# xds0112/5G_based_System_level_Integrated_Sensing_and_Communication_Simulator

Hardware: AMD Instinct MI355X
Metric: sensing slots/sec (CDL echo->2D-FFT->2D-CFAR) (higher is better)
Workload: dtype f64

## Files before the change

5g_based_system_level_integrated_sensing_and_communication_simulator_amd/_build.py:

```python
from __future__ import annotations

import os
import subprocess
import sys
from concurrent.futures import ThreadPoolExecutor

HERE = os.path.dirname(os.path.abspath(__file__))
CSRC = os.path.join(HERE, "csrc")
OBJ = os.path.join(CSRC, "build")
LIB = os.path.join(HERE, "libisac_hip.so")
SOURCES = ["capi.hip", "fft2d.hip", "tables.hip", "echo.hip", "rdm.hip", "cov.hip", "eigh.hip", "music.hip", "cdl.hip", "cdl_os.hip", "cqi.hip", "los.hip", "doa2d.hip", "doa.hip", "rxfe.hip", "targets.hip", "cfar.hip"]
HEADERS = ["isac_common.hpp", "isac_internal.hpp", "cut_window.hpp", "fft_lds.hpp", "echo_dev.hpp", "eigh_dev.hpp", "eigh_layout.hpp", os.path.join("..", "..", "include", "isac.h"), os.path.join("..", "..", "include", "isac_targets.h"), os.path.join("..", "..", "include", "isac_cfar.h"), os.path.join("..", "..", "include", "isac_cfar_mc.h")]
HIPCC = os.environ.get("HIPCC", "/opt/rocm/bin/hipcc")
FLAGS = ["--offload-arch=gfx950", "-O3", "-std=c++17", "-fPIC", "-fno-gpu-rdc", "-Wall", "-Wno-unused-function",
         "-Wno-unused-variable", "-Wno-unused-value", "-Wno-unused-result", "-ffp-contract=on"]


def _newer(target: str, deps: list[str]) -> bool:
    if not os.path.exists(target):
        return False
    t = os.path.getmtime(target)
    return all(os.path.getmtime(d) <= t for d in deps if os.path.exists(d))


def _compile(src: str, force: bool) -> str:
    obj = os.path.join(OBJ, os.path.splitext(src)[0] + ".o")
    deps = [os.path.join(CSRC, src)] + [os.path.join(CSRC, h) for h in HEADERS] + [os.path.abspath(__file__)]
    if not force and _newer(obj, deps):
        return obj
    cmd = [HIPCC, *FLAGS, "-c", os.path.join(CSRC, src), "-o", obj]
    r = subprocess.run(cmd, capture_output=True, text=True)
    if r.returncode != 0:
        raise RuntimeError(f"hipcc failed for {src}:\n{r.stdout}\n{r.stderr}")
    if r.stderr.strip():
        sys.stderr.write(r.stderr)
    return obj


def build(force: bool = False, verbose: bool = False) -> str:
    os.makedirs(OBJ, exist_ok=True)
    srcs = [s for s in SOURCES if os.path.exists(os.path.join(CSRC, s))]
    with ThreadPoolExecutor(max_workers=min(len(srcs), os.cpu_count() or 4)) as ex:
        objs = list(ex.map(lambda s: _compile(s, force), srcs))
    if force or not _newer(LIB, objs):
        cmd = [HIPCC, "--offload-arch=gfx950", "-shared", "-fPIC", "-o", LIB, *objs,
               "-Wl,-soname,libisac_hip.so", "-Wl,--no-undefined"]
        r = subprocess.run(cmd, capture_output=True, text=True)
        if r.returncode != 0:
            raise RuntimeError(f"link failed:\n{r.stdout}\n{r.stderr}")
    if verbose:
        print(f"built {LIB}")
    return LIB


if __name__ == "__main__":
    build(force="--force" in sys.argv, verbose=True)
```

5g_based_system_level_integrated_sensing_and_communication_simulator_amd/csrc/echo.hip:

```cpp
#include <cstring>
#include <type_traits>

#include "isac_internal.hpp"
#include "fft_lds.hpp"
#include "echo_dev.hpp"

namespace isac {

template <int QT, int UNROLL>
__device__ __forceinline__ void beam_sample(const c64* __restrict__ p , long long T, int A, const c64* __restrict__ s_steer , c64 (&acc)[QT]) {
#pragma unroll
  for (int q = 0; q < QT; ++q) acc[q] = mk(0.0, 0.0);
  int a = 0;
  for (; a + UNROLL <= A; a += UNROLL) {
    c64 v[UNROLL];
#pragma unroll
    for (int u = 0; u < UNROLL; ++u) v[u] = p[(long long)(a + u) * T];
#pragma unroll
    for (int u = 0; u < UNROLL; ++u)
#pragma unroll
      for (int q = 0; q < QT; ++q) acc[q] = fma(v[u], s_steer[q * A + a + u], acc[q]);
  }
  for (; a < A; ++a) {
    c64 v = p[(long long)a * T];
#pragma unroll
    for (int q = 0; q < QT; ++q) acc[q] = fma(v, s_steer[q * A + a], acc[q]);
  }
}

template <int QT, int UNROLL>
__global__ __launch_bounds__(256) void beamsum_kernel(const c64* __restrict__ tx, long long T, int A,
                                                      const c64* __restrict__ steer ,
                                                      c64* __restrict__ beam ) {
  extern __shared__ __attribute__((aligned(16))) char smem_raw[];
  c64* s_steer = reinterpret_cast<c64*>(smem_raw);
  for (int i = threadIdx.x; i < A * QT; i += blockDim.x) s_steer[i] = steer[i];
  __syncthreads();
  for (long long t0 = (long long)blockIdx.x * 256; t0 < T; t0 += (long long)gridDim.x * 256) {
    const long long t = t0 + threadIdx.x;
    const long long tc = t < T ? t : T - 1;
    c64 acc[QT];
    beam_sample<QT, UNROLL>(tx + tc, T, A, s_steer, acc);
    if (t < T) {
#pragma unroll
      for (int q = 0; q < QT; ++q) beam[(long long)q * T + t] = acc[q];
    }
  }
}

struct TargetDesc {
  double wd;
  double lsf;
  long long shift;
};
constexpr int kMaxTargets = 64;
struct TargetTable {
  TargetDesc t[kMaxTargets];
};

__device__ __forceinline__ c64 rx_phase(double w , double tt) {
  double s, c;
  sincos(w * tt, &s, &c);
  return mk(c, -s);
}

__device__ __forceinline__ c64 coef_value(c64 b, long long t, const TargetDesc& td, double w, double Ts, double tt, c64 prx) {
  double sd, cd, st, ct;
  sincos(td.wd * tt, &sd, &cd);
  sincos(w * ((double)(t - td.shift) * Ts), &st, &ct);
  c64 v = b * mk(ct, st);
  v = v * mk(cd, sd);
  v = v * td.lsf;
  return v * prx;
}

__global__ __launch_bounds__(256) void coef_kernel(const c64* __restrict__ beam, long long T, int Q,
                                                   TargetTable tab, double w , double Ts,
                                                   c64* __restrict__ coef ,
                                                   c64* __restrict__ phase_rx ) {
  long long t = (long long)blockIdx.x * blockDim.x + threadIdx.x;
  if (t >= T) return;
  double tt = (double)t * Ts;
  c64 prx = rx_phase(w, tt);
  phase_rx[t] = prx;
  for (int q = 0; q < Q; ++q) {
    long long d = tab.t[q].shift;
    c64 out = mk(0.0, 0.0);
    if (t >= d) out = coef_value(beam[(long long)q * T + (t - d)], t, tab.t[q], w, Ts, tt, prx);
    coef[(long long)q * T + t] = out;
  }
}

template <int QT>
struct CoefTargets {
  TargetDesc t[QT];
};
template <int QT, int UNROLL>
__global__ __launch_bounds__(256) void beamsum_coef_kernel(const c64* __restrict__ tx, long long T, int A,
                                                           const c64* __restrict__ steer ,
                                                           CoefTargets<QT> tab, double w , double Ts,
                                                           c64* __restrict__ coef ) {
  extern __shared__ __attribute__((aligned(16))) char smem_raw[];
  c64* s_steer = reinterpret_cast<c64*>(smem_raw);
  for (int i = threadIdx.x; i < A * QT; i += blockDim.x) s_steer[i] = steer[i];
  __syncthreads();
  for (long long t0 = (long long)blockIdx.x * 256; t0 < T; t0 += (long long)gridDim.x * 256) {
    const long long u = t0 + threadIdx.x;
    const long long uc = u < T ? u : T - 1;
    c64 acc[QT];
    beam_sample<QT, UNROLL>(tx + uc, T, A, s_steer, acc);
#pragma unroll
    for (int q = 0; q < QT; ++q) {
      const long long d = tab.t[q].shift, t = u + d;
      c64* cq = coef + (long long)q * T;
      if (u < d && u < T) cq[u] = mk(0.0, 0.0);
      if (u < T && t >= 0 && t < T) {
        const double tt = (double)t * Ts;
        cq[t] = coef_value(acc[q], t, tab.t[q], w, Ts, tt, rx_phase(w, tt));
      }
    }
  }
}

__global__ __launch_bounds__(256) void radar_waveform_kernel(long long T, int A, int Q, const c64* __restrict__ coef,
                                                             const c64* __restrict__ steer_rq ,
                                                             const c64* __restrict__ phase_rx, int noise_mode,
                                                             const c64* __restrict__ noise, double n0s, uint64_t seed,
                                                             c64* __restrict__ rx) {
  long long t = (long long)blockIdx.x * blockDim.x + threadIdx.x;
  int r = blockIdx.y;
  if (t >= T) return;
  rx[t + T * r] = rx_sample(t, r, T, Q, coef, steer_rq + (long long)r * Q, phase_rx, noise_mode, noise, n0s, seed);
}

struct OfdmGeom {
  int nfft, n_sc, cp_base, cp_long, sym_per_half;
};

template <class FFT, bool SYNTH, int QT = 0>
__global__ __launch_bounds__(256, 2) void demod_kernel(OfdmGeom g, long long T, int A, int L_whole, int L_out,
                                                       const c64* __restrict__ tw,
                                                       int Q_rt, const c64* __restrict__ coef,
                                                       const c64* __restrict__ steer_rq, const c64* __restrict__ phase_rx,
                                                       int noise_mode, const c64* __restrict__ noise, double n0s,
                                                       uint64_t seed,
                                                       const c64* __restrict__ wave,
                                                       c64* __restrict__ grid, const c64* __restrict__ logtab_g) {
  extern __shared__ __attribute__((aligned(16))) char smem_raw[];
  c64* lds = reinterpret_cast<c64*>(smem_raw);
  const int tid = threadIdx.x;
  FFT fft;
  constexpr bool kTables = SYNTH && QT > 0 && std::is_same<FFT, Fft4096>::value;
  const int Q = QT ? QT : Q_rt;
  {
    const int col = blockIdx.x;
    const int l = col % L_whole, r = col / L_whole;
    const int cp = cp_of_symbol(l, g.cp_base, g.cp_long, g.sym_per_half);
    const int off = cp / 2;
    const long long w0 = symbol_start(l, g.nfft, g.cp_base, g.cp_long, g.sym_per_half) + off;
    const int dshift = cp - off;
    if constexpr (SYNTH) {
      const c64* sr = steer_rq + (long long)r * Q;
      if (noise_mode == ISAC_NOISE_PHILOX) {
        if constexpr (kTables) {
          c64* lt = lds + FFT::LDS_ELEMS;
          if (tid < kLogTabSize) lt[tid] = logtab_g[tid];
          fft.init_table(lds, tw, tid);
          const c64* w256 = lds + FFT::IMG;
          fft.template fill<4>([&](int n) { return rx_sample(w0 + n, r, T, Q, coef, sr, phase_rx, ISAC_NOISE_PHILOX, noise, n0s, seed, w256, lt); }, tid);
          fft.init_twiddles(tw, tid);
        } else {
          fft.template fill<4>([&](int n) { return rx_sample(w0 + n, r, T, Q, coef, sr, phase_rx, ISAC_NOISE_PHILOX, noise, n0s, seed); }, tid);
        }
      } else {
        const int nm = (noise_mode == ISAC_NOISE_INJECTED) ? ISAC_NOISE_INJECTED : ISAC_NOISE_NONE;
        fft.template fill<8>([&](int n) { return rx_sample(w0 + n, r, T, Q, coef, sr, phase_rx, nm, noise, n0s, seed); }, tid);
      }
    } else {
      const c64* src = wave + w0 + T * (long long)r;
      fft.fill([&](int n) { return src[n]; }, tid);
    }
    if (!(kTables && noise_mode == ISAC_NOISE_PHILOX)) fft.init(lds, tw, tid);
    fft.template transform<-1>(lds, tw, tid);
    c64* dst = grid + (long long)g.n_sc * ((long long)l + (long long)L_out * r);
    const int half = g.n_sc / 2;
    fft.drain(
        [&](int k, c64 v) {
          const int kb = (k < g.nfft / 2) ? k : k - g.nfft;
          const int row = kb + half;
          const c64 ph = fft.phase_ramp(lds, tw, kb, dshift);
          if (row >= 0 && row < g.n_sc) {
            const c64 o = v * ph;
            __builtin_nontemporal_store(o.re, &dst[row].re);
            __builtin_nontemporal_store(o.im, &dst[row].im);
          }
        },
        tid);
  }
}

template <int QT, int NZ>
// ... 225 lines not shown
  }
}

__global__ __launch_bounds__(256) void mod_window_kernel(OfdmGeom g, ModIo io, int A, int L, const c64* __restrict__ head,
                                                         const double* __restrict__ rise, c64* __restrict__ wave) {
  const long long i = (long long)blockIdx.x * blockDim.x + threadIdx.x;
  const long long n = (long long)io.n_win * L * A;
  if (i >= n) return;
  const int w = (int)(i % io.n_win), l = (int)((i / io.n_win) % L), a = (int)(i / ((long long)io.n_win * L));
  const long long e = symbol_start(io.sym0 + l + 1, g.nfft, g.cp_base, g.cp_long, g.sym_per_half) -
                      symbol_start(io.sym0, g.nfft, g.cp_base, g.cp_long, g.sym_per_half);
  c64* p = wave + io.t_off + io.wave_rows * (long long)a + e - io.n_win + w;
  const c64 hv = head[(long long)io.n_win * ((long long)((l + 1) % L) + (long long)L * a) + w];
  *p = *p * rise[io.n_win - 1 - w] + hv;
}

__global__ __launch_bounds__(256) void copy_slot_kernel(const c64* __restrict__ src , c64* __restrict__ dst, int K, int L, int A,
                                                        int grid_cols, int l_off) {
  const long long i = (long long)blockIdx.x * blockDim.x + threadIdx.x;
  const long long n = (long long)K * L * A;
  if (i >= n) return;
  const long long k = i % K, l = (i / K) % L, a = i / ((long long)K * L);
  dst[k + (long long)K * ((l_off + l) + (long long)grid_cols * a)] = src ? src[i] : mk(0.0, 0.0);
}

__global__ __launch_bounds__(256) void synth_qpsk_kernel(c64* __restrict__ grid, int K, int L, int A, uint64_t seed,
                                                         int zero_s_slots) {
  long long i = (long long)blockIdx.x * blockDim.x + threadIdx.x;
  long long n = (long long)K * L * A;
  if (i >= n) return;
  int l = (int)((i / K) % L);
  int slot = l / 14;
  c64 v = mk(0.0, 0.0);
  if (!(zero_s_slots && (slot % 4) == 3)) {
    uint32_t o[4];
    philox4x32_10((uint32_t)i, (uint32_t)((uint64_t)i >> 32), 1u, 0u, (uint32_t)seed, (uint32_t)(seed >> 32), o);
    v = mk((o[0] & 1u) ? kR2 : -kR2, (o[1] & 1u) ? kR2 : -kR2);
  }
  grid[i] = v;
}

}

using namespace isac;

static int check_carrier(isac_ctx* ctx, const isac_carrier* c) {
  if (!c) return fail(ctx, ISAC_ERR_INVALID_ARG, "carrier is NULL");
  if (c->nfft < 128 || c->nfft > 4096 || (c->nfft & (c->nfft - 1)))
    return fail(ctx, ISAC_ERR_UNSUPPORTED, "carrier.nfft must be a power of two in 128..4096: no integral normal cyclic prefix (144 Nfft / 2048 samples) exists below 128");
  if (c->n_sc <= 0 || c->n_sc > c->nfft || (c->n_sc & 1)) return fail(ctx, ISAC_ERR_INVALID_ARG, "carrier.n_sc invalid");
  if (c->scs_khz != 15 && c->scs_khz != 30 && c->scs_khz != 60 && c->scs_khz != 120)
    return fail(ctx, ISAC_ERR_INVALID_ARG, "carrier.scs_khz must be 15/30/60/120");
  return ISAC_OK;
}

static OfdmGeom geom_of(const isac_carrier* c) {
  Numerology n = numerology(c->nfft, c->scs_khz);
  return OfdmGeom{c->nfft, c->n_sc, n.cp_base, n.cp_long, n.sym_per_half};
}

static int whole_symbols(const OfdmGeom& g, long long T) {
  long long lo = 0, hi = T / g.nfft + 1;
  while (lo < hi) {
    long long mid = (lo + hi + 1) / 2;
    if (symbol_start((int)mid, g.nfft, g.cp_base, g.cp_long, g.sym_per_half) <= T) lo = mid; else hi = mid - 1;
  }
  return (int)lo;
}

extern "C" int isac_ofdm_symbol_count(const isac_carrier* carrier, int64_t T, int32_t* n_symbols) {
  if (!carrier || !n_symbols || T < 0) return ISAC_ERR_INVALID_ARG;
  *n_symbols = whole_symbols(geom_of(carrier), T);
  return ISAC_OK;
}

extern "C" int isac_ofdm_waveform_length(const isac_carrier* carrier, int32_t L, int64_t* T) {
  if (!carrier || !T || L < 0) return ISAC_ERR_INVALID_ARG;
  OfdmGeom g = geom_of(carrier);
  *T = symbol_start(L, g.nfft, g.cp_base, g.cp_long, g.sym_per_half);
  return ISAC_OK;
}

static int prepare_echo(isac_ctx* ctx, const c64* d_tx, long long T, const isac_radar_channel_params* rp,
                        const uint8_t* los, int* q_out, bool coef_only = false) {
  if (!d_tx || !rp || !los) return fail(ctx, ISAC_ERR_INVALID_ARG, "NULL argument");
  if (T <= 0 || rp->n_ants <= 0 || rp->n_targets < 0) return fail(ctx, ISAC_ERR_INVALID_ARG, "bad T / n_ants / n_targets");
  ctx->lazy.valid = false;
  if (!(rp->fs > 0)) return fail(ctx, ISAC_ERR_INVALID_ARG, "fs must be positive");
  const int A = rp->n_ants;
  const double c0 = 299792458.0;
  const double lambda = c0 / rp->fc;
  const double Ts = 1.0 / rp->fs;
  const double two_pi = 2.0 * M_PI;
  TargetTable tab{};
  std::vector<c64> steer_aq;
  int Q = 0;
  for (int i = 0; i < rp->n_targets; ++i) {
    if (los[i] != 1) continue;
    if (Q >= kMaxTargets) return fail(ctx, ISAC_ERR_CAPACITY, "more than 64 LoS targets");
    for (int a = 0; a < A; ++a) {
      const isac_c64 sv = rp->rx_steering[(size_t)a + (size_t)A * i];
      steer_aq.push_back(mk(sv.re, sv.im));
    }
    double path_delay = 2.0 * rp->range[i] / c0;
    tab.t[Q].shift = (long long)std::ceil(path_delay / Ts);
    double fd = 2.0 * rp->velocity[i] / lambda;
    tab.t[Q].wd = two_pi * fd;
    tab.t[Q].lsf = rp->large_scale_fading[i];
    ++Q;
  }
  if (Q == 0) return fail(ctx, ISAC_ERR_NO_LOS, "no LoS target: rxWaveform is empty (basicRadarChannel.m:59,64)");
  std::vector<c64> steer_rq((size_t)A * Q);
  for (int q = 0; q < Q; ++q)
    for (int a = 0; a < A; ++a) steer_rq[(size_t)a * Q + q] = steer_aq[(size_t)q * A + a];
  ISAC_TRY(ensure(ctx, ctx->steer, sizeof(c64) * (size_t)A * Q * 2));
  ISAC_TRY(ensure(ctx, ctx->beam, sizeof(c64) * (size_t)Q * T));
  ISAC_TRY(ensure(ctx, ctx->coef, sizeof(c64) * (size_t)Q * T));
  ISAC_TRY(ensure(ctx, ctx->phase_rx, sizeof(c64) * (size_t)T));
  c64* d_steer_aq = (c64*)ctx->steer.p;
  {
    const size_t bytes = sizeof(c64) * (size_t)A * Q * 2;
    void* hst = nullptr;
    ISAC_TRY(stage_acquire(ctx, bytes, &hst));
    std::memcpy(hst, steer_aq.data(), bytes / 2);
    std::memcpy((char*)hst + bytes / 2, steer_rq.data(), bytes / 2);
    ISAC_TRY(stage_commit(ctx, d_steer_aq, bytes));
  }
  const unsigned gb = cdiv(T, 256);
  const unsigned gbs = (unsigned)std::min<long long>(gb, 1024);
  timeline_mark(ctx, 0, ctx->stream);
  const double w = two_pi * rp->fc;
  if (coef_only && Q <= 2) {
    auto launch = [&](auto qc) {
      constexpr int QT = decltype(qc)::value;
      CoefTargets<QT> ct;
      for (int q = 0; q < QT; ++q) ct.t[q] = tab.t[q];
      hipLaunchKernelGGL((beamsum_coef_kernel<QT, 32>), dim3(gbs), dim3(256), sizeof(c64) * A * QT, ctx->stream, d_tx, T, A, (const c64*)d_steer_aq, ct, w, Ts, (c64*)ctx->coef.p);
    };
    if (Q == 1) launch(std::integral_constant<int, 1>{});
    else launch(std::integral_constant<int, 2>{});
    ISAC_HIP(hipGetLastError());
    timeline_mark(ctx, 1, ctx->stream);
    *q_out = Q;
    return ISAC_OK;
  }
#define ISAC_BEAMSUM(QT) \
  hipLaunchKernelGGL((beamsum_kernel<QT, (QT <= 2 ? 32 : 8)>), dim3(gbs), dim3(256), sizeof(c64) * A * QT, ctx->stream, d_tx, T, A, st, bm)
  for (int q0 = 0; q0 < Q;) {
    int rem = Q - q0;
    const c64* st = d_steer_aq + (size_t)q0 * A;
    c64* bm = (c64*)ctx->beam.p + (size_t)q0 * T;
    if (rem >= 8) { ISAC_BEAMSUM(8); q0 += 8; }
    else if (rem >= 4) { ISAC_BEAMSUM(4); q0 += 4; }
    else if (rem >= 2) { ISAC_BEAMSUM(2); q0 += 2; }
    else { ISAC_BEAMSUM(1); q0 += 1; }
  }
#undef ISAC_BEAMSUM
  timeline_mark(ctx, 1, ctx->stream);
  hipLaunchKernelGGL(coef_kernel, dim3(gb), dim3(256), 0, ctx->stream, (const c64*)ctx->beam.p, T, Q, tab, w, Ts,
                     (c64*)ctx->coef.p, (c64*)ctx->phase_rx.p);
  ISAC_HIP(hipGetLastError());
  *q_out = Q;
  return ISAC_OK;
}

extern "C" int isac_basic_radar_channel_dev(isac_ctx* ctx, const isac_c64* d_tx_wave, int64_t T,
                                            const isac_radar_channel_params* rp, const uint8_t* los, int noise_mode,
                                            const isac_c64* d_noise_unit, uint64_t seed, isac_c64* d_rx_wave) {
  ISAC_ENTER(ctx);
  if (!d_rx_wave) return fail(ctx, ISAC_ERR_INVALID_ARG, "rx_wave is NULL");
  if (noise_mode == ISAC_NOISE_INJECTED && !d_noise_unit) return fail(ctx, ISAC_ERR_INVALID_ARG, "noise buffer missing");
  if (noise_mode < ISAC_NOISE_NONE || noise_mode > ISAC_NOISE_PHILOX)
    return fail(ctx, ISAC_ERR_INVALID_ARG, "basicRadarChannel returns a time-domain waveform: noise modes NONE / INJECTED / PHILOX only");
  int Q = 0;
  ISAC_TRY(prepare_echo(ctx, (const c64*)d_tx_wave, T, rp, los, &Q));
  const int A = rp->n_ants;
  const double n0s = std::sqrt(rp->n0 / 2.0);
  hipLaunchKernelGGL(radar_waveform_kernel, dim3(cdiv(T, 256), A), dim3(256), 0, ctx->stream, (long long)T, A, Q,
                     (const c64*)ctx->coef.p, (const c64*)ctx->steer.p + (size_t)A * Q, (const c64*)ctx->phase_rx.p,
                     noise_mode, (const c64*)d_noise_unit, n0s, seed, (c64*)d_rx_wave);
  ISAC_HIP(hipGetLastError());
  return ISAC_OK;
}

template <int MAXQ, class F>
static int echo_dispatch(int Q, F&& f) {
  if constexpr (MAXQ > 0)
    if (Q != MAXQ) return echo_dispatch<MAXQ - 1>(Q, f);
  return f(std::integral_constant<int, MAXQ>{});
}

static int padded_symbols(int L_whole, int tx_dim_l, int32_t* l_out) {
  const int L_out = L_whole < tx_dim_l ? tx_dim_l : L_whole;
  if (l_out) *l_out = L_out;
  return L_out;
}

template <class FFT, bool SYNTH, int QT = 0>
static int launch_demod(isac_ctx* ctx, const OfdmGeom& g, long long T, int A, int L_whole, int L_out, const c64* tw, int Q,
                        int noise_mode, const c64* noise, double n0s, uint64_t seed, const c64* wave, c64* grid) {
  size_t lds = sizeof(c64) * (FFT::LDS_ELEMS + kLogTabSize);
  const c64* logtab = nullptr;
  ISAC_TRY(isac_get_logtab(ctx, &logtab));
  auto kern = demod_kernel<FFT, SYNTH, QT>;
  ISAC_TRY(allow_lds(ctx, reinterpret_cast<const void*>(kern), lds));
  hipLaunchKernelGGL(kern, dim3((unsigned)(L_whole * A)) , dim3(256), lds, ctx->stream, g, T, A, L_whole, L_out, tw, Q,
                     (const c64*)ctx->coef.p, SYNTH ? (const c64*)ctx->steer.p + (size_t)A * Q : nullptr,
                     (const c64*)ctx->phase_rx.p, noise_mode, noise, n0s, seed, wave, grid, logtab);
  ISAC_HIP(hipGetLastError());
  return ISAC_OK;
}

static int spectral_prepare(isac_ctx* ctx, const c64* d_tx, long long T, const isac_radar_channel_params* rp, const uint8_t* los,
                            const OfdmGeom& g, int* q_out, int* l_whole_out, bool coef_only = false) {
  int Q = 0;
  ISAC_TRY(prepare_echo(ctx, d_tx, T, rp, los, &Q, coef_only));
  const int L_whole = whole_symbols(g, T);
  if (L_whole <= 0) return fail(ctx, ISAC_ERR_SHORT_WAVEFORM, "waveform shorter than one OFDM symbol");
  ISAC_TRY(ensure(ctx, ctx->dgrid, sizeof(c64) * (size_t)g.n_sc * L_whole * Q));
  const c64* tw = nullptr;
  ISAC_TRY(isac_get_twiddles(ctx, g.nfft, &tw));
  ISAC_FFT_DISPATCH(g.nfft, ISAC_TRY((launch_demod<FFT, false>(ctx, g, T, Q, L_whole, L_whole, tw, 0, 0, nullptr, 0.0, 0,
                                                               (const c64*)ctx->coef.p, (c64*)ctx->dgrid.p))));
  *q_out = Q;
  *l_whole_out = L_whole;
  return ISAC_OK;
}

static bool spectral_mode(int noise_mode) { return noise_mode == ISAC_NOISE_PHILOX_SPECTRAL || noise_mode == ISAC_NOISE_INJECTED_SPECTRAL; }

template <int QT>
static int launch_echo_spectral(isac_ctx* ctx, const OfdmGeom& g, int A, int L_whole, int L_out, int Q, int noise_mode,
                                const c64* noise, double sig, uint64_t seed, c64* grid) {
  const dim3 gr((unsigned)spectral_grid_size(L_whole, A)), bl(256);
  const c64* D = (const c64*)ctx->dgrid.p;
  const c64* srq = (const c64*)ctx->steer.p + (size_t)A * Q;
  auto kern = noise_mode == ISAC_NOISE_PHILOX_SPECTRAL ? echo_spectral_kernel<QT, 1> : noise_mode == ISAC_NOISE_INJECTED_SPECTRAL ? echo_spectral_kernel<QT, 2> : echo_spectral_kernel<QT, 0>;
  hipLaunchKernelGGL(kern, gr, bl, 0, ctx->stream, g.n_sc, L_whole, L_out, A, Q, D, srq, sig, seed, noise, grid);
  ISAC_HIP(hipGetLastError());
  return ISAC_OK;
}

template <class Kern, class... Args>
static int launch_echo_range(isac_ctx* ctx, Kern kern, int L_whole, int A, Args... args) {
  const size_t lds = sizeof(c64) * Fft4096W::LDS_ELEMS;
  ISAC_TRY(allow_lds(ctx, reinterpret_cast<const void*>(kern), lds));
  hipLaunchKernelGGL(kern, dim3((unsigned)spectral_grid_size(L_whole, A)), dim3(Fft4096W::NT), lds, ctx->stream, args...);
  ISAC_HIP(hipGetLastError());
  return ISAC_OK;
}

static int mono_static_spectral(isac_ctx* ctx, const c64* d_tx, long long T, int tx_dim_l, const OfdmGeom& g,
                                const isac_radar_channel_params* rp, const uint8_t* los, int noise_mode, const c64* d_noise,
                                uint64_t seed, c64* d_grid, int32_t* l_out) {
  int Q = 0, L_whole = 0;
  ISAC_TRY(spectral_prepare(ctx, d_tx, T, rp, los, g, &Q, &L_whole));
  const int A = rp->n_ants;
  const int L_out = padded_symbols(L_whole, tx_dim_l, l_out);
  if (L_out > L_whole) ISAC_HIP(hipMemsetAsync(d_grid, 0, sizeof(c64) * (size_t)g.n_sc * L_out * A, ctx->stream));
  const double sig = std::sqrt(rp->n0 / 2.0) * std::sqrt((double)g.nfft);
  return echo_dispatch<4>(Q, [&](auto qc) { return launch_echo_spectral<decltype(qc)::value>(ctx, g, A, L_whole, L_out, Q, noise_mode, d_noise, sig, seed, d_grid); });
}

extern "C" int isac_mono_static_sensing_dev(isac_ctx* ctx, const isac_c64* d_tx_wave, int64_t T, int32_t tx_dim_l,
                                            const isac_carrier* carrier, const isac_radar_channel_params* rp,
                                            const uint8_t* los, int noise_mode, const isac_c64* d_noise_unit,
                                            uint64_t seed, isac_c64* d_echo_grid, int32_t* l_out) {
  ISAC_ENTER(ctx);
  ctx->range_cache.valid = false;
  ISAC_TRY(check_carrier(ctx, carrier));
  if (!d_echo_grid) return fail(ctx, ISAC_ERR_INVALID_ARG, "echo_grid is NULL");
  if ((noise_mode == ISAC_NOISE_INJECTED || noise_mode == ISAC_NOISE_INJECTED_SPECTRAL) && !d_noise_unit)
    return fail(ctx, ISAC_ERR_INVALID_ARG, "noise buffer missing");
  if (noise_mode < ISAC_NOISE_NONE || noise_mode > ISAC_NOISE_INJECTED_SPECTRAL) return fail(ctx, ISAC_ERR_INVALID_ARG, "unknown noise mode");
  if (spectral_mode(noise_mode))
    return mono_static_spectral(ctx, (const c64*)d_tx_wave, T, tx_dim_l, geom_of(carrier), rp, los, noise_mode, (const c64*)d_noise_unit,
                                seed, (c64*)d_echo_grid, l_out);
  int Q = 0;
  ISAC_TRY(prepare_echo(ctx, (const c64*)d_tx_wave, T, rp, los, &Q));
  OfdmGeom g = geom_of(carrier);
  const int A = rp->n_ants;
  const int L_whole = whole_symbols(g, T);
  if (L_whole <= 0) return fail(ctx, ISAC_ERR_SHORT_WAVEFORM, "waveform shorter than one OFDM symbol");
  const int L_out = padded_symbols(L_whole, tx_dim_l, l_out);
  if (L_out > L_whole) ISAC_HIP(hipMemsetAsync(d_echo_grid, 0, sizeof(c64) * (size_t)g.n_sc * L_out * A, ctx->stream));
  const c64* tw = nullptr;
  ISAC_TRY(isac_get_twiddles(ctx, g.nfft, &tw));
  const double n0s = std::sqrt(rp->n0 / 2.0);
  if (g.nfft == 4096)
    return echo_dispatch<4>(Q, [&](auto qc) {
      return launch_demod<Fft4096, true, decltype(qc)::value>(ctx, g, T, A, L_whole, L_out, tw, Q, noise_mode, (const c64*)d_noise_unit, n0s, seed, nullptr, (c64*)d_echo_grid);
    });
  ISAC_FFT_DISPATCH(g.nfft, ISAC_TRY((launch_demod<FFT, true>(ctx, g, T, A, L_whole, L_out, tw, Q, noise_mode,
                                                              (const c64*)d_noise_unit, n0s, seed, nullptr,
                                                              (c64*)d_echo_grid))));
  return ISAC_OK;
}

extern "C" int isac_mono_static_sensing_fused_dev(isac_ctx* ctx, const isac_c64* d_tx_wave, int64_t T, int32_t tx_dim_l,
// ... 206 lines not shown
```

5g_based_system_level_integrated_sensing_and_communication_simulator_amd/csrc/isac_common.hpp:

```cpp
#pragma once

#include <hip/hip_runtime.h>

#include <array>
#include <cmath>
#include <cstdint>
#include <cstdio>
#include <cstdlib>
#include <cstring>
#include <map>
#include <string>
#include <type_traits>
#include <utility>
#include <vector>

#include "../../include/isac.h"
#include "cut_window.hpp"

namespace isac {

struct __attribute__((aligned(16))) c64 {
  double re, im;
};
static_assert(sizeof(c64) == 16, "c64 must match isac_c64 / MATLAB interleaved complex");

__host__ __device__ inline c64 mk(double r, double i) { return c64{r, i}; }
__host__ __device__ inline c64 operator+(c64 a, c64 b) { return {a.re + b.re, a.im + b.im}; }
__host__ __device__ inline c64 operator-(c64 a, c64 b) { return {a.re - b.re, a.im - b.im}; }
__host__ __device__ inline c64 operator*(c64 a, c64 b) {
  return {a.re * b.re - a.im * b.im, a.re * b.im + a.im * b.re};
}
__host__ __device__ inline c64 operator*(c64 a, double s) { return {a.re * s, a.im * s}; }
__host__ __device__ inline c64 operator*(double s, c64 a) { return {a.re * s, a.im * s}; }
__host__ __device__ inline c64 conj(c64 a) { return {a.re, -a.im}; }
__host__ __device__ inline c64 mul_conj(c64 a, c64 b) {
  return {a.re * b.re + a.im * b.im, a.im * b.re - a.re * b.im};
}
__host__ __device__ inline c64 mul_i(c64 a) { return {-a.im, a.re}; }
__host__ __device__ inline c64 mul_mi(c64 a) { return {a.im, -a.re}; }
__host__ __device__ inline c64& operator+=(c64& a, c64 b) { a.re += b.re; a.im += b.im; return a; }
__host__ __device__ inline c64 fma(c64 a, c64 b, c64 c) {
  return {::fma(a.re, b.re, ::fma(-a.im, b.im, c.re)), ::fma(a.re, b.im, ::fma(a.im, b.re, c.im))};
}

typedef unsigned int u32x4_t __attribute__((ext_vector_type(4)));
constexpr int kBufferRsrcFlags = 0x00020000;
__device__ __forceinline__ __amdgpu_buffer_rsrc_t buffer_of(const void* base, unsigned bytes) {
  const unsigned long long b = reinterpret_cast<unsigned long long>(base);
  const unsigned lo = __builtin_amdgcn_readfirstlane((unsigned)b), hi = __builtin_amdgcn_readfirstlane((unsigned)(b >> 32));
  void* ub = reinterpret_cast<void*>(((unsigned long long)hi << 32) | lo);
  return __builtin_amdgcn_make_buffer_rsrc(ub, 0, (int)__builtin_amdgcn_readfirstlane(bytes), kBufferRsrcFlags);
}
__device__ __forceinline__ c64 buffer_load_c64(__amdgpu_buffer_rsrc_t rs, unsigned byte_off) {
  return __builtin_bit_cast(c64, __builtin_amdgcn_raw_buffer_load_b128(rs, (int)byte_off, 0, 0));
}
__device__ __forceinline__ void buffer_store_c64_nt(__amdgpu_buffer_rsrc_t rs, unsigned byte_off, c64 v) {
  __builtin_amdgcn_raw_buffer_store_b128(__builtin_bit_cast(u32x4_t, v), rs, (int)byte_off, 0,  2);
}

template <hipError_t (*Free)(void*)>
struct OwnedBuf {
  void* p = nullptr;
  size_t cap = 0;
  OwnedBuf() = default;
  OwnedBuf(OwnedBuf&& o) noexcept : p(o.p), cap(o.cap) { o.p = nullptr; o.cap = 0; }
  OwnedBuf& operator=(OwnedBuf&& o) noexcept { if (this != &o) { (void)reset(); p = o.p; cap = o.cap; o.p = nullptr; o.cap = 0; } return *this; }
  OwnedBuf(const OwnedBuf&) = delete;
  OwnedBuf& operator=(const OwnedBuf&) = delete;
  ~OwnedBuf() { (void)reset(); }
  hipError_t reset() {
    const hipError_t e = p ? Free(p) : hipSuccess;
    p = nullptr;
    cap = 0;
    return e;
  }
};
using DevBuf = OwnedBuf<hipFree>;
using PinnedBuf = OwnedBuf<hipHostFree>;
static_assert(!std::is_copy_constructible<DevBuf>::value && std::is_nothrow_move_constructible<DevBuf>::value, "one owner per allocation");

enum TableKind { kTwiddle, kW512Pack, kLogTab, kKaiser3, kKaiser3Shifted, kRiseWindow, kSind, kDoa2d };
struct TableKey {
  TableKind kind;
  std::array<long long, 4> par{};
  bool operator<(const TableKey& o) const { return kind != o.kind ? kind < o.kind : par < o.par; }
};

struct Fft2dLast {
  bool valid = false;
  std::vector<int32_t> det_rc;
  std::vector<double> det_pow;
  std::vector<int32_t> ant_off;
  std::vector<double> spectrum_db;
  std::vector<double> range_db, velocity_db;
};

struct RangeCache {
  bool valid = false;
  const void* rx = nullptr;
  const void* tx = nullptr;
// ... 217 lines not shown
  ISAC_TRY(bounce_ready(ctx, bytes));
  const bool two = ctx->bounce.cap >= 2 * kBounceChunk;
  size_t pend_off[2] = {0, 0}, pend_n[2] = {0, 0};
  int half = 0;
  for (size_t off = 0; off < bytes; off += kBounceChunk, half ^= 1) {
    const size_t n = bytes - off < kBounceChunk ? bytes - off : kBounceChunk;
    const int h = two ? half : 0;
    char* b = (char*)ctx->bounce.p + (size_t)h * kBounceChunk;
    if (pend_n[h]) { ISAC_HIP(hipEventSynchronize(ctx->ev_bounce[h])); std::memcpy((char*)dst + pend_off[h], b, pend_n[h]); pend_n[h] = 0; }
    ISAC_HIP(hipMemcpyAsync(b, (const char*)src + off, n, hipMemcpyDeviceToHost, ctx->stream));
    ISAC_HIP(hipEventRecord(ctx->ev_bounce[h], ctx->stream));
    pend_off[h] = off; pend_n[h] = n;
  }
  ISAC_HIP(hipStreamSynchronize(ctx->stream));
  for (int h = 0; h < 2; ++h) if (pend_n[h]) std::memcpy((char*)dst + pend_off[h], (char*)ctx->bounce.p + (size_t)h * kBounceChunk, pend_n[h]);
  return ISAC_OK;
}

inline int upload(isac_ctx* ctx, DevBuf& b, const void* src, size_t bytes) {
  ISAC_TRY(ensure(ctx, b, bytes));
  ISAC_TRY(copy_h2d(ctx, b.p, src, bytes));
  return ISAC_OK;
}

inline int stage_acquire(isac_ctx* ctx, size_t bytes, void** host) {
  StageSlot& sl = ctx->stage_ring[ctx->stage_next];
  if (!sl.ev) ISAC_HIP(hipEventCreateWithFlags(&sl.ev, hipEventDisableTiming));
  if (sl.busy) { ISAC_HIP(hipEventSynchronize(sl.ev)); sl.busy = false; }
  if (sl.mem.cap < bytes) ISAC_TRY(ensure_pinned_buf(ctx, sl.mem, bytes < 65536 ? 65536 : bytes));
  *host = sl.mem.p;
  return ISAC_OK;
}
inline int stage_commit(isac_ctx* ctx, void* d_dst, size_t bytes) {
  StageSlot& sl = ctx->stage_ring[ctx->stage_next];
  ISAC_HIP(hipMemcpyAsync(d_dst, sl.mem.p, bytes, hipMemcpyHostToDevice, ctx->stream));
  ISAC_HIP(hipEventRecord(sl.ev, ctx->stream));
  sl.busy = true;
  ctx->stage_next = (ctx->stage_next + 1) % kStageSlots;
  return ISAC_OK;
}
inline int stage_upload(isac_ctx* ctx, void* d_dst, const void* src, size_t bytes) {
  void* h = nullptr;
  ISAC_TRY(stage_acquire(ctx, bytes, &h));
  std::memcpy(h, src, bytes);
  return stage_commit(ctx, d_dst, bytes);
}
struct MetaPack {
  size_t align;
  std::vector<char> host;
  explicit MetaPack(size_t align_ = 64) : align(align_) {}
  size_t add(const void* src, size_t bytes) {
    const size_t off = host.size();
    host.resize(off + (bytes + align - 1) / align * align, 0);
    if (bytes) std::memcpy(host.data() + off, src, bytes);
    return off;
  }
  template <class T>
  size_t add(const std::vector<T>& v) { return add(v.data(), sizeof(T) * v.size()); }
  int upload(isac_ctx* ctx, DevBuf& b) {
    ISAC_TRY(ensure(ctx, b, host.size() + 64));
    return stage_upload(ctx, b.p, host.data(), host.size());
  }
};

inline int profile_begin(isac_ctx* ctx) {
  if (ctx->profile) ISAC_HIP(hipEventRecord(ctx->ev_k0, ctx->stream));
  return ISAC_OK;
}
inline int profile_end(isac_ctx* ctx) {
  if (ctx->profile) { ISAC_HIP(hipEventRecord(ctx->ev_k1, ctx->stream)); ctx->profile_recorded = true; }
  return ISAC_OK;
}

inline int ctx_n_cus(isac_ctx* ctx, int* n_cus) {
  if (ctx->n_cus <= 0) {
    int v = 0;
    ISAC_HIP(hipDeviceGetAttribute(&v, hipDeviceAttributeMultiprocessorCount, ctx->device));
    ctx->n_cus = v > 0 ? v : 256;
  }
  *n_cus = ctx->n_cus;
  return ISAC_OK;
}

struct Numerology {
  int nfft, mu, cp_base, cp_long, sym_per_half;
};
inline Numerology numerology(int nfft, int scs_khz) {
  Numerology n{};
  n.nfft = nfft;
  n.mu = 0;
  for (int s = scs_khz / 15; s > 1; s >>= 1) n.mu++;
  double scale = nfft / 2048.0;
  n.cp_base = (int)std::lround(144.0 * scale);
  n.cp_long = n.cp_base + (int)std::lround(16.0 * scale * (1 << n.mu));
  n.sym_per_half = 7 * (1 << n.mu);
  return n;
}
__host__ __device__ inline int cp_of_symbol(int l, int cp_base, int cp_long, int sym_per_half) {
  return (l % sym_per_half) == 0 ? cp_long : cp_base;
}
__host__ __device__ inline long long symbol_start(int l, int nfft, int cp_base, int cp_long, int sym_per_half) {
  long long n_long = (l + sym_per_half - 1) / sym_per_half;
  return (long long)l * (nfft + cp_base) + n_long * (cp_long - cp_base);
}

inline unsigned cdiv(long long a, long long b) { return (unsigned)((a + b - 1) / b); }

}
```

Measured before the change: 21290.

## Beam-sum only samples read by demod FFT windows and pass steering by kernel argument

```diff
diff --git a/5g_based_system_level_integrated_sensing_and_communication_simulator_amd/_build.py b/5g_based_system_level_integrated_sensing_and_communication_simulator_amd/_build.py
--- a/5g_based_system_level_integrated_sensing_and_communication_simulator_amd/_build.py
+++ b/5g_based_system_level_integrated_sensing_and_communication_simulator_amd/_build.py
@@ -10,7 +10,7 @@
 OBJ = os.path.join(CSRC, "build")
 LIB = os.path.join(HERE, "libisac_hip.so")
 SOURCES = ["capi.hip", "fft2d.hip", "tables.hip", "echo.hip", "rdm.hip", "cov.hip", "eigh.hip", "music.hip", "cdl.hip", "cdl_os.hip", "cqi.hip", "los.hip", "doa2d.hip", "doa.hip", "rxfe.hip", "targets.hip", "cfar.hip"]
-HEADERS = ["isac_common.hpp", "isac_internal.hpp", "cut_window.hpp", "fft_lds.hpp", "echo_dev.hpp", "eigh_dev.hpp", "eigh_layout.hpp", os.path.join("..", "..", "include", "isac.h"), os.path.join("..", "..", "include", "isac_targets.h"), os.path.join("..", "..", "include", "isac_cfar.h"), os.path.join("..", "..", "include", "isac_cfar_mc.h")]
+HEADERS = ["isac_common.hpp", "isac_internal.hpp", "cut_window.hpp", "ofdm_symbol.hpp", "beam_window.hpp", "fft_lds.hpp", "echo_dev.hpp", "eigh_dev.hpp", "eigh_layout.hpp", os.path.join("..", "..", "include", "isac.h"), os.path.join("..", "..", "include", "isac_targets.h"), os.path.join("..", "..", "include", "isac_cfar.h"), os.path.join("..", "..", "include", "isac_cfar_mc.h")]
 HIPCC = os.environ.get("HIPCC", "/opt/rocm/bin/hipcc")
 FLAGS = ["--offload-arch=gfx950", "-O3", "-std=c++17", "-fPIC", "-fno-gpu-rdc", "-Wall", "-Wno-unused-function",
          "-Wno-unused-variable", "-Wno-unused-value", "-Wno-unused-result", "-ffp-contract=on"]
diff --git a/5g_based_system_level_integrated_sensing_and_communication_simulator_amd/csrc/beam_window.hpp b/5g_based_system_level_integrated_sensing_and_communication_simulator_amd/csrc/beam_window.hpp
--- /dev/null
+++ b/5g_based_system_level_integrated_sensing_and_communication_simulator_amd/csrc/beam_window.hpp
@@ -0,0 +1,54 @@
+#pragma once
+
+#include "ofdm_symbol.hpp"
+
+namespace isac {
+
+constexpr int kBeamUnit = 256;
+constexpr int kBeamLine = 8;
+
+struct BeamWindow {
+  int nfft, cp_base, cp_long, sym_per_half;
+  int n_sym;
+  int units_per_symbol;
+  long long T, d_min, d_max;
+};
+
+ISAC_HD inline long long bw_floor_line(long long u) { return u & ~(long long)(kBeamLine - 1); }
+ISAC_HD inline int bw_symbols(const BeamWindow& w) { return w.n_sym > 0 ? w.n_sym : 1; }
+ISAC_HD inline long long bw_units(const BeamWindow& w) { return (long long)bw_symbols(w) * w.units_per_symbol; }
+
+ISAC_HD inline long long bw_window_start(const BeamWindow& w, int l) {
+  return symbol_start(l, w.nfft, w.cp_base, w.cp_long, w.sym_per_half) + cp_of_symbol(l, w.cp_base, w.cp_long, w.sym_per_half) / 2;
+}
+ISAC_HD inline long long bw_range_start(const BeamWindow& w, int l) { return (w.n_sym > 0 ? bw_window_start(w, l) : 0) - w.d_max; }
+ISAC_HD inline long long bw_range_end(const BeamWindow& w, int l) {
+  if (w.n_sym <= 0) return w.T;
+  const long long e = bw_window_start(w, l) + w.nfft - w.d_min;
+  return e < w.T ? e : w.T;
+}
+ISAC_HD inline long long bw_first(const BeamWindow& w, int l) {
+  const long long s = bw_range_start(w, l);
+  if (l == 0) return s;
+  const long long p = bw_range_end(w, l - 1);
+  return s > p ? s : p;
+}
+ISAC_HD inline long long bw_sample(const BeamWindow& w, int l, int j, int i) {
+  const long long s = bw_range_start(w, l), u = bw_floor_line(s) + (long long)j * kBeamUnit + i;
+  return u < s ? u + (long long)w.units_per_symbol * kBeamUnit : u;
+}
+
+inline BeamWindow beam_window(int nfft, int cp_base, int cp_long, int sym_per_half, int n_sym, long long T, long long d_min, long long d_max) {
+  BeamWindow w{nfft, cp_base, cp_long, sym_per_half, n_sym, 0, T, d_min, d_max};
+  auto units = [](long long span) { return (span + (kBeamUnit - 1)) / kBeamUnit; };
+  const long long per_symbol = units(nfft + (d_max - d_min)), whole = units(T + d_max);
+  if (n_sym > 0 && per_symbol * n_sym < whole) {
+    w.units_per_symbol = (int)per_symbol;
+  } else {
+    w.n_sym = 0;
+    w.units_per_symbol = whole > 1 ? (int)whole : 1;
+  }
+  return w;
+}
+
+}
diff --git a/5g_based_system_level_integrated_sensing_and_communication_simulator_amd/csrc/echo.hip b/5g_based_system_level_integrated_sensing_and_communication_simulator_amd/csrc/echo.hip
--- a/5g_based_system_level_integrated_sensing_and_communication_simulator_amd/csrc/echo.hip
+++ b/5g_based_system_level_integrated_sensing_and_communication_simulator_amd/csrc/echo.hip
@@ -4,6 +4,7 @@
 #include "isac_internal.hpp"
 #include "fft_lds.hpp"
 #include "echo_dev.hpp"
+#include "beam_window.hpp"
 
 namespace isac {
 
@@ -95,28 +96,51 @@
 struct CoefTargets {
   TargetDesc t[QT];
 };
+constexpr int kSteerArgMax = 128;
+struct SteerArg {
+  c64 v[kSteerArgMax];
+};
 template <int QT, int UNROLL>
 __global__ __launch_bounds__(256) void beamsum_coef_kernel(const c64* __restrict__ tx, long long T, int A,
                                                            const c64* __restrict__ steer ,
-                                                           CoefTargets<QT> tab, double w , double Ts,
+                                                           const SteerArg steer_arg, c64* __restrict__ steer_out ,
+                                                           BeamWindow bw, CoefTargets<QT> tab, double w , double Ts,
                                                            c64* __restrict__ coef ) {
   extern __shared__ __attribute__((aligned(16))) char smem_raw[];
   c64* s_steer = reinterpret_cast<c64*>(smem_raw);
-  for (int i = threadIdx.x; i < A * QT; i += blockDim.x) s_steer[i] = steer[i];
+  if (steer) {
+    for (int i = threadIdx.x; i < A * QT; i += blockDim.x) s_steer[i] = steer[i];
+  } else {
+    for (int i = threadIdx.x; i < A * QT; i += blockDim.x) {
+      const c64 v = steer_arg.v[i];
+      s_steer[i] = v;
+      if (blockIdx.x == 0) {
+        const int q = i / A, a = i - q * A;
+        steer_out[i] = v;
+        steer_out[A * QT + a * QT + q] = v;
+      }
+    }
+  }
   __syncthreads();
-  for (long long t0 = (long long)blockIdx.x * 256; t0 < T; t0 += (long long)gridDim.x * 256) {
-    const long long u = t0 + threadIdx.x;
-    const long long uc = u < T ? u : T - 1;
+  const int n_units = (int)bw_units(bw);
+  for (int k = blockIdx.x; k < n_units; k += gridDim.x) {
+    const int l = k / bw.units_per_symbol, j = k - l * bw.units_per_symbol;
+    const long long lo = bw_first(bw, l), hi = bw_range_end(bw, l);
+    const long long u = bw_sample(bw, l, j, threadIdx.x);
+    const bool mine = u >= lo && u < hi;
+    if (!__any(mine)) continue;
+    long long uc = u < lo ? lo : u < hi ? u : hi - 1;
+    uc = uc < 0 ? 0 : uc < T ? uc : T - 1;
     c64 acc[QT];
     beam_sample<QT, UNROLL>(tx + uc, T, A, s_steer, acc);
+    if (!mine) continue;
 #pragma unroll
     for (int q = 0; q < QT; ++q) {
-      const long long d = tab.t[q].shift, t = u + d;
+      const long long t = u + tab.t[q].shift;
       c64* cq = coef + (long long)q * T;
-      if (u < d && u < T) cq[u] = mk(0.0, 0.0);
-      if (u < T && t >= 0 && t < T) {
+      if (t >= 0 && t < T) {
         const double tt = (double)t * Ts;
-        cq[t] = coef_value(acc[q], t, tab.t[q], w, Ts, tt, rx_phase(w, tt));
+        cq[t] = u < 0 ? mk(0.0, 0.0) : coef_value(acc[q], t, tab.t[q], w, Ts, tt, rx_phase(w, tt));
       }
     }
   }
@@ -508,7 +532,7 @@
 }
 
 static int prepare_echo(isac_ctx* ctx, const c64* d_tx, long long T, const isac_radar_channel_params* rp,
-                        const uint8_t* los, int* q_out, bool coef_only = false) {
+                        const uint8_t* los, int* q_out, const OfdmGeom* coef_only = nullptr) {
   if (!d_tx || !rp || !los) return fail(ctx, ISAC_ERR_INVALID_ARG, "NULL argument");
   if (T <= 0 || rp->n_ants <= 0 || rp->n_targets < 0) return fail(ctx, ISAC_ERR_INVALID_ARG, "bad T / n_ants / n_targets");
   ctx->lazy.valid = false;
@@ -544,7 +568,9 @@
   ISAC_TRY(ensure(ctx, ctx->coef, sizeof(c64) * (size_t)Q * T));
   ISAC_TRY(ensure(ctx, ctx->phase_rx, sizeof(c64) * (size_t)T));
   c64* d_steer_aq = (c64*)ctx->steer.p;
-  {
+  const bool one_launch = coef_only && Q <= 2;
+  const bool steer_by_arg = one_launch && A * Q <= kSteerArgMax;
+  if (!steer_by_arg) {
     const size_t bytes = sizeof(c64) * (size_t)A * Q * 2;
     void* hst = nullptr;
     ISAC_TRY(stage_acquire(ctx, bytes, &hst));
@@ -556,12 +582,22 @@
   const unsigned gbs = (unsigned)std::min<long long>(gb, 1024);
   timeline_mark(ctx, 0, ctx->stream);
   const double w = two_pi * rp->fc;
-  if (coef_only && Q <= 2) {
+  if (one_launch) {
+    long long d_min = tab.t[0].shift, d_max = d_min;
+    for (int q = 1; q < Q; ++q) { d_min = std::min(d_min, tab.t[q].shift); d_max = std::max(d_max, tab.t[q].shift); }
+    const OfdmGeom& g = *coef_only;
+    constexpr long long kSpan = 1LL << 38;
+    if (T >= kSpan || d_max >= kSpan || d_min <= -kSpan) return fail(ctx, ISAC_ERR_CAPACITY, "waveform or target delay beyond the beam-sum's unit count");
+    const BeamWindow bw = beam_window(g.nfft, g.cp_base, g.cp_long, g.sym_per_half, whole_symbols(g, T), T, d_min, d_max);
+    const unsigned gbu = (unsigned)std::max<long long>(1, std::min<long long>(bw_units(bw), 1024));
+    SteerArg sa{};
+    if (steer_by_arg) std::memcpy(sa.v, steer_aq.data(), sizeof(c64) * (size_t)A * Q);
     auto launch = [&](auto qc) {
       constexpr int QT = decltype(qc)::value;
       CoefTargets<QT> ct;
       for (int q = 0; q < QT; ++q) ct.t[q] = tab.t[q];
-      hipLaunchKernelGGL((beamsum_coef_kernel<QT, 32>), dim3(gbs), dim3(256), sizeof(c64) * A * QT, ctx->stream, d_tx, T, A, (const c64*)d_steer_aq, ct, w, Ts, (c64*)ctx->coef.p);
+      hipLaunchKernelGGL((beamsum_coef_kernel<QT, 32>), dim3(gbu), dim3(256), sizeof(c64) * A * QT, ctx->stream, d_tx, T, A, steer_by_arg ? nullptr : (const c64*)d_steer_aq, sa,
+                         d_steer_aq, bw, ct, w, Ts, (c64*)ctx->coef.p);
     };
     if (Q == 1) launch(std::integral_constant<int, 1>{});
     else launch(std::integral_constant<int, 2>{});
@@ -640,7 +676,7 @@
 static int spectral_prepare(isac_ctx* ctx, const c64* d_tx, long long T, const isac_radar_channel_params* rp, const uint8_t* los,
                             const OfdmGeom& g, int* q_out, int* l_whole_out, bool coef_only = false) {
   int Q = 0;
-  ISAC_TRY(prepare_echo(ctx, d_tx, T, rp, los, &Q, coef_only));
+  ISAC_TRY(prepare_echo(ctx, d_tx, T, rp, los, &Q, coef_only ? &g : nullptr));
   const int L_whole = whole_symbols(g, T);
   if (L_whole <= 0) return fail(ctx, ISAC_ERR_SHORT_WAVEFORM, "waveform shorter than one OFDM symbol");
   ISAC_TRY(ensure(ctx, ctx->dgrid, sizeof(c64) * (size_t)g.n_sc * L_whole * Q));
diff --git a/5g_based_system_level_integrated_sensing_and_communication_simulator_amd/csrc/isac_common.hpp b/5g_based_system_level_integrated_sensing_and_communication_simulator_amd/csrc/isac_common.hpp
--- a/5g_based_system_level_integrated_sensing_and_communication_simulator_amd/csrc/isac_common.hpp
+++ b/5g_based_system_level_integrated_sensing_and_communication_simulator_amd/csrc/isac_common.hpp
@@ -16,6 +16,7 @@
 
 #include "../../include/isac.h"
 #include "cut_window.hpp"
+#include "ofdm_symbol.hpp"
 
 namespace isac {
 
@@ -399,27 +400,6 @@
   return ISAC_OK;
 }
 
-struct Numerology {
-  int nfft, mu, cp_base, cp_long, sym_per_half;
-};
-inline Numerology numerology(int nfft, int scs_khz) {
-  Numerology n{};
-  n.nfft = nfft;
-  n.mu = 0;
-  for (int s = scs_khz / 15; s > 1; s >>= 1) n.mu++;
-  double scale = nfft / 2048.0;
-  n.cp_base = (int)std::lround(144.0 * scale);
-  n.cp_long = n.cp_base + (int)std::lround(16.0 * scale * (1 << n.mu));
-  n.sym_per_half = 7 * (1 << n.mu);
-  return n;
-}
-__host__ __device__ inline int cp_of_symbol(int l, int cp_base, int cp_long, int sym_per_half) {
-  return (l % sym_per_half) == 0 ? cp_long : cp_base;
-}
-__host__ __device__ inline long long symbol_start(int l, int nfft, int cp_base, int cp_long, int sym_per_half) {
-  long long n_long = (l + sym_per_half - 1) / sym_per_half;
-  return (long long)l * (nfft + cp_base) + n_long * (cp_long - cp_base);
-}
 
 inline unsigned cdiv(long long a, long long b) { return (unsigned)((a + b - 1) / b); }
 
diff --git a/5g_based_system_level_integrated_sensing_and_communication_simulator_amd/csrc/ofdm_symbol.hpp b/5g_based_system_level_integrated_sensing_and_communication_simulator_amd/csrc/ofdm_symbol.hpp
--- /dev/null
+++ b/5g_based_system_level_integrated_sensing_and_communication_simulator_amd/csrc/ofdm_symbol.hpp
@@ -0,0 +1,35 @@
+#pragma once
+
+#include <cmath>
+
+#if defined(__HIPCC__)
+#define ISAC_HD __host__ __device__
+#else
+#define ISAC_HD
+#endif
+
+namespace isac {
+
+struct Numerology {
+  int nfft, mu, cp_base, cp_long, sym_per_half;
+};
+inline Numerology numerology(int nfft, int scs_khz) {
+  Numerology n{};
+  n.nfft = nfft;
+  n.mu = 0;
+  for (int s = scs_khz / 15; s > 1; s >>= 1) n.mu++;
+  double scale = nfft / 2048.0;
+  n.cp_base = (int)std::lround(144.0 * scale);
+  n.cp_long = n.cp_base + (int)std::lround(16.0 * scale * (1 << n.mu));
+  n.sym_per_half = 7 * (1 << n.mu);
+  return n;
+}
+ISAC_HD inline int cp_of_symbol(int l, int cp_base, int cp_long, int sym_per_half) {
+  return (l % sym_per_half) == 0 ? cp_long : cp_base;
+}
+ISAC_HD inline long long symbol_start(int l, int nfft, int cp_base, int cp_long, int sym_per_half) {
+  long long n_long = (l + sym_per_half - 1) / sym_per_half;
+  return (long long)l * (nfft + cp_base) + n_long * (cp_long - cp_base);
+}
+
+}
```

Result: faster. 21940, median of 6 (+3.1%).
